# JustinPrivitera/Real_Time_Ray_Tracer

Hardware: AMD Instinct MI355X
Metric: Mrays/s + ms/frame at 3840x2160, 16 AO samples, 64 spheres; 1/2/4/8 GPU (higher is better)
Workload: dtype f32

## Files before the change

### __graft_entry__.py

```python
from __future__ import annotations

import os
import subprocess
import sys
from pathlib import Path

ROOT = Path(__file__).resolve().parent


def build() -> None:
    env = dict(os.environ)
    env.setdefault("PYTORCH_ROCM_ARCH", "gfx950")
    jobs = str(min(16, os.cpu_count() or 1))
    subprocess.run(["make", "-j", jobs, "lib", "headless", "oracle"], cwd=ROOT, check=True, env=env)
    if str(ROOT) not in sys.path:
        sys.path.insert(0, str(ROOT))
    import real_time_ray_tracer_amd as rt

    rt.load()


def smoke() -> None:
    if str(ROOT) not in sys.path:
        sys.path.insert(0, str(ROOT))
    import numpy as np

    import oracle
    import real_time_ray_tracer_amd as rt

    W, H, spp = 64, 48, 4
    h = rt.Header.synthetic(16, spp, 1234, rt.aspect_for(W, H))
    r = rt.Renderer(W, H, h.S, h.AA, device=0)
    ho = h.copy()
    s = rt.SSBO(ho, W, H)
    d = oracle.dims(W, H, h.S, h.AA)
    img = np.zeros((H, W, 4), np.float32)
    fg = fo = 0
    for k in range(3):
        h.fill_rand_buffer(7000 + k)
        h.set_mode(fg, h.num_objects)
        r.upload_header(h)
        fg = r.dispatch(rt.host._lib.RT_MODE_AO_PP, fg)
        s.set_header(h)
        fo = oracle.dispatch(s.data, d, 1, fo, img)
    g = r.download()
    r.close()
    ok = np.abs(g.image - img) <= 1e-4 * np.maximum(np.abs(g.image), np.abs(img)) + 1e-6
    if not ok.all() or fg != fo:
        raise RuntimeError(f"smoke: {int((~ok).sum())} image values differ from the oracle")
    if not np.array_equal(g.depth.view(np.uint32), s.depth.view(np.uint32)):
        raise RuntimeError("smoke: depth g-buffer differs from the oracle")
    print(f"smoke ok: {W}x{H} mode 1, 3 frames, image mean {img[..., :3].mean():.4f}")


if __name__ == "__main__":
    build()
    if len(sys.argv) > 1 and sys.argv[1] == "smoke":
        smoke()
```

### real_time_ray_tracer_amd/csrc/rt_kernels_impl.h

```cpp
#pragma once
#include <hip/hip_runtime.h>

#include "rt_device.h"
#include "rt_kernels.h"

namespace rt {

namespace {

constexpr int kBlock = 256;
constexpr float kGamma = 1.0f / 2.2f;

__device__ __forceinline__ void stage_shapes(const FrameParams& P, float4* lds) {
  const int n = P.nobj;
  for (int k = threadIdx.x; k < 4 * n; k += blockDim.x) {
    int tab = k / n, i = k - tab * n;
    lds[k] = P.shapes[(size_t)tab * P.S + i];
  }
}

__device__ __forceinline__ f3 primary_dir(const FrameParams& P, float hp, float vp) {
  f3 a = mk(P.lx + hp * P.hx, P.ly + hp * P.hy, P.lz + hp * P.hz);
  return normalize(mk(a.x + vp * P.vx, a.y + vp * P.vy, a.z + vp * P.vz));
}
// ... 726 lines not shown
        bounce_round<PL>(P, geo, n, light, live, pos, dir, perm, t, ind, lit);
      }
      if (live) live = !segment(seg, t, ind, lit);
    }
    if (P.tile_cost && (threadIdx.x & 63) == 0)
      P.tile_cost[((unsigned)by * gridDim.x + (unsigned)bx) * (BWX * BWY) + (threadIdx.x >> 6)] = (unsigned)rounds;
  } else {
    for (int seg = 0; active && seg < P.D; ++seg) {
      float t;
      const int ind = closest_hit<ALLSPH>(geo, geo2, n, pos, dir, 0.001f, t);
      const bool lit = ind == -1 || shadow_lit<ALLSPH>(geo, geo2, n, light, pos + t * dir);
      if (segment(seg, t, ind, lit)) break;
    }
  }
  count_work(P, active, y, nseg, nshadow);
  if (active) store_color(P, fd.out_pix, fd.image, x, y, gamma_out(0.0f + rr, 0.0f + rg, 0.0f + rb));
  if (ABL == 7) {
    const unsigned mx = wave_max(active ? nseg : 0u);
    const unsigned long long tend = __builtin_amdgcn_s_memrealtime();
    if ((threadIdx.x & 63) == 0 && active)
      P.out_pix[(size_t)(y - P.band_row0) * P.W + x] =
          make_float4(__uint_as_float((unsigned)tstart), __uint_as_float((unsigned)tend), __uint_as_float(mx),
                      __uint_as_float((unsigned)(tstart >> 32)));
  }
}

template <bool ALLSPH, bool PL = false, bool LT = false, int ABL = 0, int BWX = 2, int BWY = 2, bool MF = true>
__global__ __launch_bounds__(64 * BWX * BWY) void hybrid_kernel(const unsigned* __restrict__ tord,
                                                                const float4* __restrict__ gsph,
                                                                const float4* __restrict__ gshp, unsigned gx,
                                                                FrameParams P) {
  extern __shared__ float4 lds[];
  __shared__ int hperm[64 * BWX * BWY];
  if (!ALLSPH || LT) {
    if (LT) stage_tables(P, lds);
    else stage_shapes(P, lds);
    __syncthreads();
  }
  if constexpr (kHybridTilesPerBlock == 2) {
    const unsigned gx = gridDim.x, gy = (unsigned)(P.trace_rows + 8 * BWY - 1) / (8 * BWY), n = gx * gy;
    const unsigned b = blockIdx.x + blockIdx.y * gx;
#pragma unroll 1
    for (int t = 0; t < 2; ++t) {
      const unsigned u = t == 0 ? b : n - 1 - b;
      if (b > n - 1 - b || (t == 1 && u == b)) break;
      unsigned bx = u % gx, by = u / gx;
      if (tord) {
        const unsigned v = tord[u];
        bx = v & 0xffffu;
        by = v >> 16;
      }
      hybrid_tile<ALLSPH, PL, LT, ABL, BWX, BWY>(P, lds, hperm + 64 * (threadIdx.x >> 6), bx, by, frame_dst(P, blockIdx.z), gsph, gshp);
    }
  } else if constexpr (kHybridTilesPerBlock > 1) {
#pragma unroll 1
    for (int t = 0; t < kHybridTilesPerBlock; ++t)
      hybrid_tile<ALLSPH, PL, LT, ABL, BWX, BWY>(P, lds, hperm + 64 * (threadIdx.x >> 6), blockIdx.x,
                                                 blockIdx.y * kHybridTilesPerBlock + t, frame_dst(P, blockIdx.z), gsph, gshp);
  } else if constexpr (kHybridFramesPerBlock == 1) {
    const bool pre = !MF && ALLSPH && !LT;
    float4 g0;
    if (pre) g0 = gsph[threadIdx.x & 63];
    unsigned bx = blockIdx.x, by = blockIdx.y;
    if (tord) {
      const unsigned t = tord[blockIdx.x + blockIdx.y * gx];
      bx = t & 0xffffu;
      by = t >> 16;
    }
    hybrid_tile<ALLSPH, PL, LT, ABL, BWX, BWY>(P, lds, hperm + 64 * (threadIdx.x >> 6), bx, by,
                                               frame_dst<MF>(P, blockIdx.z), gsph, gshp, pre ? &g0 : nullptr);
  } else {
    int j0;
    const int nj = block_frames<kHybridFramesPerBlock>(P, j0);
#pragma unroll 1
    for (int j = 0; j < nj; ++j)
      hybrid_tile<ALLSPH, PL, LT, ABL, BWX, BWY>(P, lds, hperm + 64 * (threadIdx.x >> 6), blockIdx.x, blockIdx.y,
                                                 frame_dst(P, j0 + j), gsph, gshp);
  }
}

enum { PRIM_HIT = 0, PRIM_MISS = 1, PRIM_EMISSIVE = 2 };

struct BatchLds {
  int prec, sres, pstop, pkind, perm, cmask, rls, geol, total;
};
__host__ __device__ constexpr BatchLds batch_lds(int spp, int pool, int ntail, bool rls_lds = true) {
  const int TP = pool / spp > 0 ? pool / spp : 1, NS = TP * spp;
  BatchLds L{};
  L.prec = 0;
  L.sres = 16 * TP;
  L.pstop = L.sres + 12 * NS;
  L.pkind = L.pstop + 4 * TP;
  L.perm = L.pkind + 4 * ((TP + 1) & ~1);
  L.cmask = (L.perm + 256 + 7) & ~7;
  L.rls = (L.cmask + 8 * 32 + 15) & ~15;
  L.geol = L.rls + (rls_lds ? 32 * spp : 0);
  L.total = L.geol + 16 * ntail;
  return L;
}

#ifndef RT_AO_MINW
#define RT_AO_MINW 7
#endif
#ifndef RT_PT_WIDE
#define RT_PT_WIDE 1
#endif
#ifndef RT_B1_DEFER
#define RT_B1_DEFER 1
#endif
#ifndef RT_B1_PRIO
#define RT_B1_PRIO 1
#endif
#ifndef RT_START_PRIO
#define RT_START_PRIO 1
#endif
#ifndef RT_B1_CREAD
#define RT_B1_CREAD 1
#endif
constexpr int kAoMinWaves = RT_AO_MINW;
template <int MINW, bool LAZY = true, int POOL = kPool, int ABL = 0, bool TAIL = false, bool B1 = false,
          int SPPC = 0, bool PT = false, bool CNT = true, bool PL = false, bool MF = false, bool CL = true, int DC = 0,
          bool CLON = false, bool PTW = false>
__global__ __launch_bounds__(64, MINW) void ao_batch_kernel(FrameParams P, const float4* __restrict__ geo) {
  if (RT_START_PRIO) __builtin_amdgcn_s_setprio(1);
  unsigned long long* const cnts = CNT ? P.counters : nullptr;
  unsigned long long* const rowc = CNT ? P.row_counters : nullptr;
  extern __shared__ float4 lds[];
  const int spp = SPPC ? SPPC : P.spp, W = P.W, D = DC ? DC : P.D, nobj = P.nobj;
  const bool use_cl = CL && (CLON || P.ncl > 0);
  const int fj = MF ? (int)blockIdx.y : 0;
  const int fslot = MF ? (P.mf_slot0 + fj) % P.F : 0;
  float4* const f_nrm = MF ? (float4*)P.hist_nrm[fslot] : P.nrm;
  float4* const f_dep = MF ? (float4*)P.hist_dep[fslot] : P.dep;
  const float4* const f_nrm_prev = MF ? f_nrm : P.nrm_prev;
  const float4* const f_dep_prev = MF ? f_dep : P.dep_prev;
  float4* const f_out = MF ? (float4*)P.hist_pix[fslot] : P.out_pix;
  float4* const f_img = MF ? (fj == P.mf_n - 1 ? P.image : nullptr) : P.image;
  const float4* const f_rb = MF ? P.mf_rb + (size_t)fj * 2 * spp : P.rb;
  const int TP = POOL / spp > 0 ? POOL / spp : 1;
  const int lane = threadIdx.x;
  const int NS = TP * spp;
  const BatchLds LO = batch_lds(spp, POOL, 0, !PTW);
  char* lbase = (char*)lds;
  float4* prec = (float4*)(lbase + LO.prec);
  float* sres = (float*)(lbase + LO.sres);
  int* pstop = (int*)(lbase + LO.pstop);
  int* pkind = (int*)(lbase + LO.pkind);
  int* perm = (int*)(lbase + LO.perm);
  unsigned long long* cmask = (unsigned long long*)(lbase + LO.cmask);
  float4* rls = (float4*)(lbase + LO.rls);
  if (!PTW)
    for (int k = lane; k < 2 * spp; k += 64) rls[k] = f_rb[k];
  for (int k = lane; k < TP; k += 64) pstop[k] = -1;
  float4* geol = (float4*)(lbase + LO.geol);
  constexpr bool tail_lds = TAIL && PT && !PTW;
  const bool tail_ok = TAIL;
  const float4* const tgeo = tail_lds ? geol : geo;
  const bool pt_ok = PT && B1 && (tail_lds || PTW);
  bool geol_valid = false;
  if (tail_lds && !pt_ok) {
    for (int k = lane; k < nobj; k += 64) geol[k] = geo[k];
    geol_valid = true;
  }
  const float4* const clus = geo + (size_t)3 * P.S;
  const unsigned long long* const clm = (const unsigned long long*)(geo + (size_t)3 * P.S + kMaxClusters);
  auto col_at = [&](int ind) -> float4 {
    int o = ind - P.S;
    asm("" : "+v"(o));
    return geo[o - P.S];
  };
  auto aux_at = [&](int ind) -> float4 {
    int o = ind - P.S;
    asm("" : "+v"(o));
    return geo[o];
  };

  const long long npix = (long long)P.trace_rows * W;
  unsigned pb = blockIdx.x;
  if (P.pool_rot > 0) {
    const unsigned Q = (unsigned)P.pool_rot, r = pb / Q;
    if ((r + 1) * Q <= gridDim.x) {
      unsigned c = pb - r * Q + r % Q;
      c = c >= Q ? c - Q : c;
      pb = r * Q + c;
    }
  }
  const long long p0 = (long long)pb * TP;
  const int np = (int)(npix - p0 < TP ? npix - p0 : TP);
  const int total = np * spp;

  unsigned long long tsec[8] = {0, 0, 0, 0, 0, 0, 0, 0};
  constexpr bool kLaps = ABL == 3 || ABL == 6 || ABL == 8;
  unsigned long long tmark = kLaps ? __builtin_amdgcn_s_memtime() : 0;
  auto lap = [&](int k) {
    if (kLaps) {
      unsigned long long now = __builtin_amdgcn_s_memtime();
      tsec[k] += now - tmark;
      tmark = now;
    }
  };
  const int yf = P.trace_row0 + (int)(p0 / W), xf = (int)(p0 % W);
  auto pool_xy = [&](int lp, int& x, int& y) {
    int xi = xf + lp;
    y = yf;
    if (xi >= W) {
      int q = (int)((unsigned)xi / (unsigned)W);
      y += q;
      xi -= q * W;
    }
    x = xi;
  };
  const int yl = P.trace_row0 + (int)((p0 + np - 1) / W), xl = (int)((p0 + np - 1) % W);
  int ncull = 0;
  const int nwords = (nobj + 63) >> 6;
  unsigned long long pmask = 0;
  {
    const ConeF cone = pool_cone_f(P, yf == yl ? xf : 0, yf == yl ? xl : W - 1, yf, yl);
    for (int w = 0; w < nwords; ++w) {
      int i = (w << 6) + lane;
      bool keep = i < nobj && !cone_misses_f(cone, geo[i], P.cx, P.cy, P.cz);
      if (PL) keep = keep && geo[i].x == geo[i].x;
      unsigned long long m = __ballot(keep);
      ncull += __popcll(m);
      if (lane == 0) cmask[w] = m;
    }
    if (PL) {
      pmask = plane_cone_mask(P, cone, mk(P.cx, P.cy, P.cz));
      ncull += __popcll(pmask) + (P.nplanes > 64 ? P.nplanes - 64 : 0);
    }
  }
  __syncthreads();
// ... 40 lines not shown
  unsigned nseg = 0;
  unsigned long long exec_tests = 0;

  const float inv_spp = P.inv_spp;
  auto div_spp = [&](int it) { return SPPC ? (int)((unsigned)it / (unsigned)SPPC) : (int)(((float)it + 0.5f) * inv_spp); };
  auto finish = [&](int it, float r, float g, float b, float stopv, int segs) {
    sres[it] = r;
    sres[NS + it] = g;
    sres[2 * NS + it] = b;
    if (stopv >= 0.0f) {
      const int lq = div_spp(it);
      atomicMax(&pstop[lq], ((it - lq * spp) << 16) | (int)stopv);
    }
    if (rowc) {
      int x, y;
      pool_xy(div_spp(it), x, y);
      atomicAdd(&rowc[y - P.band_row0],
                (unsigned long long)(kSetupCost + ncull + (segs >= 2 ? b1cost + (segs - 2) * nobj : 0)));
    }
  };

  auto shade = [&](int ind, float t, f3& ps, f3& dr, f3 hm, float& r, float& g, float& b, int dpt, int it,
                   bool first) -> bool {
    const int lp = div_spp(it), aa = it - lp * spp;
    float4 att = col_at(ind);
    int kind = PRIM_MISS;
    bool go = false;
    if (ind != -1) {
      const float4 ax = aux_at(ind);
      float4 gc = make_float4(0.0f, 0.0f, 0.0f, 0.0f);
      if (!PL) {
        gc = geo[ind];
        asm volatile("" ::"v"(gc.x), "v"(gc.y), "v"(gc.z));
      }
      if (ax.x > 0.9f) {
        kind = PRIM_EMISSIVE;
      } else {
        kind = PRIM_HIT;
        f3 curr = cam + t * dr;
        f3 nn;
        if (PL) {
          const float4 gi = P.shapes[ind];
          nn = __float_as_int(P.shapes[P.S + ind].w) == SHAPE_PLANE ? xyz(gi) : normalize(curr - xyz(gi));
        } else {
          nn = normalize(curr - xyz(gc));
        }
        if (aa == 0 && first) prec[lp] = make_float4(nn.x, nn.y, nn.z, t);
        if (ABL == 9) {
          float z;
          asm volatile("v_mov_b32 %0, 0" : "=v"(z));
          const f3 c2 = cam + (t + z) * dr;
          const f3 n2 = normalize(c2 - (PL ? xyz(P.shapes[ind]) : xyz(gc)));
          const float d2 = dot(dr, n2);
          const f3 R2 = normalize(mk(dr.x - 2.0f * (d2 * n2.x), dr.y - 2.0f * (d2 * n2.y), dr.z - 2.0f * (d2 * n2.z)));
          const f3 X2 = normalize(ax.y > 0.999f ? hm + n2 : R2 + ax.y * hm);
          if (__float_as_uint(X2.x + X2.y + X2.z) == 0x7fc00001u) t = X2.x;
        }
        ps = curr;
        const float reflect = ax.y;
        f3 X;
        if (reflect > 0.999f) {
          X = hm + nn;
        } else {
          float dn = dot(dr, nn);
          f3 R = normalize(mk(dr.x - 2.0f * (dn * nn.x), dr.y - 2.0f * (dn * nn.y), dr.z - 2.0f * (dn * nn.z)));
          X = R + reflect * hm;
        }
        dr = normalize(X);
        go = dpt - 1 != 0;
      }
    }
    r = r * att.x; g = g * att.y; b = b * att.z;
    if (aa == 0 && first) pkind[lp] = kind;
    if (!go) finish(it, r, g, b, kind == PRIM_HIT ? -1.0f : (float)(D - dpt), kind == PRIM_HIT ? D : D - dpt + 1);
    return go;
  };

  auto prepare = [&]() {
    bitem = next + lane;
    bool live = false;
    if (ABL == 3) { tsec[6] += (unsigned long long)ncull; tsec[7] += 1; }
    exec_tests += (unsigned long long)ncull;
    if (bitem < total) {
      const int lp = div_spp(bitem), aa = bitem - lp * spp;
      int x, y;
      pool_xy(lp, x, y);
      const float px = (float)x, py = (float)y;
      float hp, vp;
      {
        float4 f = rbuf[2 * aa], s = rbuf[2 * aa + 1];
        float uw[2];
        grandom_n<2>({((s.x + px * f.z) - px) + f.x, s.z * px - (f.x * px) * f.z},
                     {((f.y + py * s.w) - py) + s.y, f.w * py - (s.y * py) * s.w}, uw);
        if (ABL == 4) {
          float z, uw2[2];
          asm volatile("v_mov_b32 %0, 0" : "=v"(z));
          grandom_n<2>({((s.x + px * f.z) - px) + f.x + z, s.z * px - (f.x * px) * f.z + z},
                       {((f.y + py * s.w) - py) + s.y, f.w * py - (s.y * py) * s.w}, uw2);
          if (__float_as_uint(uw2[0]) == 0x7fc00001u && __float_as_uint(uw2[1]) == 0x7fc00001u) uw[0] = uw2[0];
        }
        float u = uw[0], w = uw[1];
        normalize2(u, w);
        const float jx = aa == 0 ? 0.0f : div_rn_by(u, 6.0f, kInv6) - 0.08333f;
        const float jy = aa == 0 ? 0.0f : div_rn_by(w, 6.0f, kInv6) - 0.08333f;
        hp = div_rn_by(px + jx, P.fW, P.inv_W);
        vp = div_rn_by(py + jy, P.fH, P.inv_H);
      }
      bdir = primary_dir(P, hp, vp);
      if (ABL == 10) {
        float z;
        asm volatile("v_mov_b32 %0, 0" : "=v"(z));
        float u2 = hp + z, w2 = vp + z;
        normalize2(u2, w2);
        const float jx2 = aa == 0 ? 0.0f : div_rn_by(u2, 6.0f, kInv6) - 0.08333f;
        const float jy2 = aa == 0 ? 0.0f : div_rn_by(w2, 6.0f, kInv6) - 0.08333f;
        const f3 d2 = primary_dir(P, div_rn_by(px + jx2, P.fW, P.inv_W), div_rn_by(py + jy2, P.fH, P.inv_H));
        if (__float_as_uint(d2.x + d2.y + d2.z) == 0x7fc00001u) bdir.x = d2.y;
      }
      auto hemisphere = [&]() {
        float4 f = rbuf[2 * aa], s = rbuf[2 * aa + 1];
        float abe[3];
        grandom_n<3>({f.x + px * s.z, f.z - px * s.z, s.x * px + s.z}, {f.y + py * s.w, f.w - py * s.w, s.y * py + s.w},
                     abe);
        if (ABL == 4) {
          float z, abe2[3];
          asm volatile("v_mov_b32 %0, 0" : "=v"(z));
          grandom_n<3>({f.x + px * s.z + z, f.z - px * s.z + z, s.x * px + s.z + z},
                       {f.y + py * s.w, f.w - py * s.w, s.y * py + s.w}, abe2);
          if (__float_as_uint(abe2[0]) == 0x7fc00001u && __float_as_uint(abe2[2]) == 0x7fc00001u) abe[1] = abe2[1];
        }
        return normalize(mk(abe[0] * 2.0f - 1.0f, abe[1] * 2.0f - 1.0f, abe[2] * 2.0f - 1.0f));
      };
      if (!LAZY) bhemi = hemisphere();
      f3 cv = cam;
      asm("" : "+v"(cv.x), "+v"(cv.y), "+v"(cv.z));
      bpos = cv;
      br = bg = bb = 1.0f;
      float t = -1.0f;
      int ind = -1;
      for (int w = 0; w < nwords; ++w) {
        unsigned long long m = cmask[w];
        m = ((unsigned long long)__builtin_amdgcn_readfirstlane((unsigned)(m >> 32)) << 32) |
            (unsigned)__builtin_amdgcn_readfirstlane((unsigned)m);
        const float4* const gw = geo + (w << 6);
        while (m) {
          const unsigned j = (unsigned)pop_lowest(m);
          const int i = (w << 6) + (int)j;
          sphere_candidate(bpos, bdir, gw[j], i, 0.0001f, t, ind);
          if (ABL == 2) {
            float z;
            asm volatile("v_mov_b32 %0, 0" : "=v"(z));
            float t2 = -1.0f;
            int i2 = -1;
            sphere_candidate(mk(bpos.x + z, bpos.y, bpos.z), bdir, geo[i], i, 0.0001f, t2, i2);
            if (i2 == 0x7fffffff) t = t2;
          }
        }
      }
      if (PL) plane_pass_masked(P, pmask, bpos, bdir, 0.0001f, t, ind);
      ++nseg;
      if (LAZY && ind != -1) bhemi = hemisphere();
      live = shade(ind, t, bpos, bdir, bhemi, br, bg, bb, D, bitem, true);
    }
    bdepth = D - 1;
    b1cost = nobj;
    if (B1) {
      const unsigned long long lm1 = __ballot(live);
      if (lm1 != 0 && __popcll(lm1) >= P.b1_min) {
        lap(1);
        if (RT_B1_PRIO) __builtin_amdgcn_s_setprio(1);
        const ConeB cb = bounce_cone(live, bpos, bdir, lm1);
        float t = -1.0f;
        int ind = -1;
        b1cost = 0;
        if (ABL == 12) {
          float z;
          asm volatile("v_mov_b32 %0, 0" : "=v"(z));
          const ConeB c2 = bounce_cone(live, mk(bpos.x + z, bpos.y, bpos.z), bdir, lm1);
          unsigned long long acc = 0;
          for (int w = 0; w < nwords; ++w) {
            const int i = (w << 6) + lane_id_here();
            float4 pt;
            const bool k2 = i < nobj && bounce_cone_keep_pt(c2, geo[i], pt);
            acc ^= __ballot(k2 && pt.w != 7.0f);
          }
          if (acc == 0x123456789abcdefull) b1cost = 1;
        }
        unsigned long long ru = 0;
        int ksel = 0;
        f3 tdir = bdir;
        if (RT_B1_DEFER && !live) tdir = mk(__int_as_float(0x7fc00000), __int_as_float(0x7fc00000), __int_as_float(0x7fc00000));
        auto flush = [&]() {
          const float4 gs = geo[ksel];
          sphere_candidate_if(bpos, bdir, gs, ksel, 0.0001f, t, ind, ru);
          ru = 0;
        };
        for (int w = 0; w < nwords; ++w) {
          const int i = (w << 6) + lane_id_here();
          bool keep;
          if (pt_ok) {
            float4 pt;
            keep = i < nobj && bounce_cone_keep_pt(cb, geo[i], pt);
            if (i < nobj) geol[PTW ? i - (w << 6) : i] = pt;
          } else {
            keep = i < nobj && !bounce_cone_misses(cb, geo[i]);
          }
          if (PL) keep = keep && geo[i].x == geo[i].x;
          unsigned long long m = __ballot(keep);
          m = ((unsigned long long)__builtin_amdgcn_readfirstlane((unsigned)(m >> 32)) << 32) |
              (unsigned)__builtin_amdgcn_readfirstlane((unsigned)m);
          exec_tests += (unsigned long long)__popcll(m);
          b1cost += __popcll(m);
          if (ABL == 3) tsec[6] += (unsigned long long)__popcll(m) << 24;
          if (pt_ok) {
            geol_valid = false;
            __syncthreads();
            if (ABL == 6) lap(5);
            const float4* const qw = geol + (PTW ? 0 : (w << 6));
            const float4* const gw = geo + (w << 6);
            int qbase;
            asm("v_mov_b32 %0, %1" : "=v"(qbase) : "s"((int)(size_t)((const char*)qw - lbase)));
            if (RT_B1_DEFER || live)
              while (m) {
                const int j = pop_lowest(m), k = (w << 6) + j;
#if RT_B1_CREAD
                const float4 q = *(const float4*)(lbase + (qbase + (j << 4)));
#else
                typedef float v4f __attribute__((ext_vector_type(4)));
                v4f qv;
                int j_addr_scratch;
                asm volatile("v_lshl_add_u32 %1, %2, 4, %3\n\tds_read_b128 %0, %1\n\ts_waitcnt lgkmcnt(0)"
                             : "=v"(qv), "=&v"(j_addr_scratch)
                             : "s"(j), "v"(qbase));
                const float4 q = make_float4(qv.x, qv.y, qv.z, qv.w);
#endif
                const float4 g = gw[j];
                if (ABL == 7) {
                  const bool pass = fmaf(bdir.z, q.z, fmaf(bdir.y, q.y, bdir.x * q.x)) >= q.w;
                  const f3 pmc = bpos - xyz(g);
                  const float bb = dot(bdir, pmc);
                  const float del = fmaf(g.w, g.w, fmaf(bb, bb, -dot(pmc, pmc)));
                  const unsigned long long pm = __ballot(pass), dm = __ballot(pass && del >= 0.0f);
                  tsec[0] += 1; tsec[1] += pm != 0; tsec[2] += dm != 0;
                  tsec[3] += (unsigned long long)__popcll(pm);
                }
                const bool pass = fmaf(tdir.z, q.z, fmaf(tdir.y, q.y, tdir.x * q.x)) >= q.w;
                if (ABL == 5) {
                  float z, t2 = t;
                  int i2 = ind;
                  asm volatile("v_mov_b32 %0, 0" : "=v"(z));
                  const bool pass2 = fmaf(bdir.z + z, q.z, fmaf(bdir.y, q.y, bdir.x * q.x)) >= q.w;
                  const unsigned long long pm2 = __builtin_amdgcn_ballot_w64(pass2);
                  if (pm2 != 0) sphere_candidate_if(mk(bpos.x + z, bpos.y, bpos.z), bdir, g, k, 0.0001f, t2, i2, pm2);
                  if (i2 == 0x7fffffff) t = t2;
                }
                const unsigned long long pm = __builtin_amdgcn_ballot_w64(pass);
                if (RT_B1_DEFER) {
                  if (pm != 0) {
                    if (pm & ru) flush();
                    ru |= pm;
                    int kv = k;
                    asm("v_cndmask_b32_e64 %0, %1, %2, %3" : "=v"(ksel) : "v"(ksel), "v"(kv), "s"(pm));
                  }
                } else if (pm != 0) {
                  sphere_candidate_if(bpos, bdir, g, k, 0.0001f, t, ind, pm);
                }
              }
            if (ABL == 6) lap(6);
          } else if (live) {
            while (m) {
              const int k = (w << 6) + __builtin_ctzll(m);
              m &= m - 1;
              sphere_candidate(bpos, bdir, geo[k], k, 0.0001f, t, ind);
            }
          }
        }
        if (RT_B1_DEFER && ru != 0) flush();
        if (RT_B1_PRIO) __builtin_amdgcn_s_setprio(0);
        if (ABL == 7) { tsec[4] += 1; tsec[5] += (unsigned long long)__popcll(lm1); }
        if (live) {
          if (PL) plane_pass(P, bpos, bdir, 0.0001f, t, ind);
          ++nseg;
          live = shade(ind, t, bpos, bdir, bhemi, br, bg, bb, D - 1, bitem, false);
        }
        if (ABL == 6) lap(7);
        bdepth = D - 2;
        lap(4);
      }
    }
    unsigned long long lm = __ballot(live);
    if (live) perm[__builtin_amdgcn_mbcnt_hi((unsigned)(lm >> 32), __builtin_amdgcn_mbcnt_lo((unsigned)lm, 0u))] = lane;
    nlive = __popcll(lm);
    cursor = 0;
    next = next + 64 < total ? next + 64 : total;
    __syncthreads();
  };

  for (;;) {
    for (;;) {
      unsigned long long need = __ballot(!has);
      if (need == 0) break;
      if (cursor >= nlive) {
        if (next >= total) break;
        lap(2);
        prepare();
        lap(1);
        continue;
      }
      int r = __builtin_amdgcn_mbcnt_hi((unsigned)(need >> 32), __builtin_amdgcn_mbcnt_lo((unsigned)need, 0u));
      int take = __popcll(need) < nlive - cursor ? __popcll(need) : nlive - cursor;
      bool get = !has && r < take;
      int src = get ? perm[cursor + r] : lane;
      float sx = __shfl(bpos.x, src), sy = __shfl(bpos.y, src), sz = __shfl(bpos.z, src);
      float dx = __shfl(bdir.x, src), dy = __shfl(bdir.y, src), dz = __shfl(bdir.z, src);
      float hx = __shfl(bhemi.x, src), hy = __shfl(bhemi.y, src), hz = __shfl(bhemi.z, src);
      float cr = __shfl(br, src), cg = __shfl(bg, src), cb = __shfl(bb, src);
      int ci = __shfl(bitem, src);
      if (ABL == 11) {
        int zi;
        asm volatile("v_mov_b32 %0, 0" : "=v"(zi));
        const int s2 = src + zi;
        float q = __shfl(bpos.x, s2) + __shfl(bpos.y, s2) + __shfl(bpos.z, s2) + __shfl(bdir.x, s2) + __shfl(bdir.y, s2) +
                  __shfl(bdir.z, s2) + __shfl(bhemi.x, s2) + __shfl(bhemi.y, s2) + __shfl(bhemi.z, s2) + __shfl(br, s2) +
                  __shfl(bg, s2) + __shfl(bb, s2) + (float)__shfl(bitem, s2);
        if (__float_as_uint(q) == 0x7fc00001u) cr = q;
      }
      if (get) {
        pos = mk(sx, sy, sz);
        dir = mk(dx, dy, dz);
        hemi = mk(hx, hy, hz);
        rr = cr; rg = cg; rb = cb;
        item = ci;
        depth = bdepth;
        has = true;
      }
      cursor += take;
    }
    const unsigned long long hm = __ballot(has);
    if (hm == 0) break;
    lap(2);
    if (ABL == 3) tsec[5] += 1;
    const int L = __popcll(hm);
    if (tail_ok && next >= total && cursor >= nlive && L <= 32) {
      if (tail_lds && !geol_valid) {
        __syncthreads();
        for (int k = lane_id_here(); k < nobj; k += 64) geol[k] = geo[k];
        geol_valid = true;
      }
      int c = 0;
      while ((1 << c) < L) ++c;
      const int G = 64 >> c;
      const int rk = __builtin_amdgcn_mbcnt_hi((unsigned)(hm >> 32), __builtin_amdgcn_mbcnt_lo((unsigned)hm, 0u));
      if (has) perm[rk] = lane;
      __syncthreads();
      const int g = lane / G, pl = lane - g * G;
      const bool act = g < L;
      const int owner = act ? perm[g] : lane;
      const f3 o = mk(__shfl(pos.x, owner), __shfl(pos.y, owner), __shfl(pos.z, owner));
      const f3 d = mk(__shfl(dir.x, owner), __shfl(dir.y, owner), __shfl(dir.z, owner));
      float t = -1.0f;
      int ind = -1;
      if (use_cl && G <= kClusterTailMaxG) {
        unsigned long long kc = 0;
        for (int c0 = 0; c0 < P.ncl; c0 += G) {
          const int c = c0 + pl;
          const bool may = act && c < P.ncl && cluster_may_hit(o, d, clus[c]);
          unsigned long long b = __builtin_amdgcn_ballot_w64(may);
          for (int sh = 32; sh >= G; sh >>= 1) b |= b >> sh;
          kc |= (G == 64 ? b : (b & ((1ull << G) - 1))) << c0;
        }
        unsigned char* list = (unsigned char*)cmask;
        int cnt = 0;
        for (int w = 0; w < nwords; ++w) {
          unsigned long long m = clm[w];
          for (unsigned long long k2 = kc; k2;) m |= clm[(size_t)(1 + pop_lowest(k2)) * kClusterWords + w];
          const int ln = lane_id_here();
          if ((m >> ln) & 1ull)
            list[cnt + __builtin_amdgcn_mbcnt_hi((unsigned)(m >> 32), __builtin_amdgcn_mbcnt_lo((unsigned)m, 0u))] =
                (unsigned char)((w << 6) + ln);
          cnt += __popcll(m);
// ... 377 lines not shown
    case 9: out[i] = det_sin(__uint_as_float(__float_as_uint(in[0]) + (unsigned)i)); break;
    case 1: out[i] = grandom(in[2 * i], in[2 * i + 1]); break;
    case 2: out[i] = sqrt_rn(in[i]); break;
    case 6: {
      const unsigned per = (unsigned)in[0];
      unsigned bad = 0;
      for (unsigned k = 0; k < per; ++k) {
        unsigned long long u = (unsigned long long)i * per + k;
        if (u > 0x7f800000ull) break;
        float x = __uint_as_float((unsigned)u);
        bad += __float_as_uint(sqrt_rn(x)) != __float_as_uint(sqrtf(x));
      }
      out[i] = (float)bad;
      break;
    }
    case 7: {
      const unsigned per = (unsigned)in[0];
      unsigned bad = 0;
      for (unsigned k = 0; k < per; ++k) {
        unsigned long long u = (unsigned long long)i * per + k;
        if (u > 0x7f800000ull) break;
        float x = __uint_as_float((unsigned)u);
        bad += __float_as_uint(inv_len_rn(x)) != __float_as_uint(1.0f / sqrtf(x));
        if (u >= 0x00800000ull && u <= 0x7e800000ull) bad += __float_as_uint(rcp_rn_normal(x)) != __float_as_uint(1.0f / x);
      }
      out[i] = (float)bad;
      break;
    }
    case 8: {
      const unsigned per = (unsigned)in[0];
      unsigned bad = 0;
      for (unsigned k = 0; k < per; ++k) {
        unsigned long long u = (unsigned long long)i * per + k;
        if (u > 0x7f7fffffull) break;
        float x = __uint_as_float((unsigned)u);
        const float s = sqrt_rn_tail(x);
        if (u >= 0x0f800000ull) bad += __float_as_uint(s) != __float_as_uint(sqrtf(x));
        else bad += !(s >= 0.0f && s <= 0x1p-47f);
      }
      out[i] = (float)bad;
      break;
    }
    case 3: out[i] = in[2 * i] / in[2 * i + 1]; break;
    case 11: {
      if (i < (size_t)kSinTableN) {
        const float x = __uint_as_float(kSinTableX[i]);
        out[2 * i] = sin_ambiguous(sin_binary64(x)) ? 1.0f : 0.0f;
        out[2 * i + 1] = __uint_as_float(kSinTableX[i]);
      } else {
        out[2 * i] = -1.0f;
        out[2 * i + 1] = 0.0f;
      }
      break;
    }
    case 10: {
      const f3 lv = mk(in[4 * i], in[4 * i + 1], in[4 * i + 2]);
      const f3 l = normalize(lv);
      const float len = sqrtf(dot(lv, lv));
      const bool occ = shadow_occludes(in[4 * i + 3], l, (double)len, shadow_bounds(l, len));
      out[5 * i] = l.x; out[5 * i + 1] = l.y; out[5 * i + 2] = l.z; out[5 * i + 3] = len;
      out[5 * i + 4] = occ ? 1.0f : 0.0f;
      break;
    }
    case 4: {
      f3 v = normalize(mk(in[3 * i], in[3 * i + 1], in[3 * i + 2]));
      out[3 * i] = v.x; out[3 * i + 1] = v.y; out[3 * i + 2] = v.z;
      break;
    }
    case 5: {
      const float* a = in + 10 * i;
      out[i] = sphere_eval(mk(a[0], a[1], a[2]), mk(a[3], a[4], a[5]), make_float4(a[6], a[7], a[8], a[9]));
      break;
    }
    default: break;
  }
}

size_t shapes_lds_bytes(const FrameParams& p) { return (size_t)4 * p.nobj * sizeof(float4); }
size_t tab_lds_bytes(const FrameParams& p) { return (size_t)5 * (p.nobj > 0 ? p.nobj : 1) * sizeof(float4); }

}

constexpr int kRefDepth = 20;

template <int SPPC, bool PL, int DC = 0, bool CLON = false>
inline void launch_batch(bool tl, bool cnt, dim3 g, dim3 b, size_t lds, hipStream_t stream, const FrameParams& q) {
  constexpr bool GT = RT_GLOBAL_TAIL;
  constexpr bool TLC = RT_TL_CLUSTERS;
  constexpr bool PTWV = RT_PT_WIDE;
  if (q.mf_n > 0) {
    g.y = (unsigned)q.mf_n;
    if (tl)
      hipLaunchKernelGGL((ao_batch_kernel<kAoMinWaves, true, kPool, 0, true, true, SPPC, true, false, PL, true, TLC, DC, CLON>), g, b, lds, stream, q, q.sph);
    else
      hipLaunchKernelGGL((ao_batch_kernel<kAoMinWaves, true, kPool, 0, GT, true, SPPC, PTWV, false, PL, true, true, DC, CLON, PTWV>), g, b, lds, stream, q, q.sph);
    return;
  }
  if (tl && cnt)
    hipLaunchKernelGGL((ao_batch_kernel<kAoMinWaves, true, kPool, 0, true, true, SPPC, true, true, PL, false, TLC, DC, CLON>), g, b, lds, stream, q, q.sph);
  else if (tl)
    hipLaunchKernelGGL((ao_batch_kernel<kAoMinWaves, true, kPool, 0, true, true, SPPC, true, false, PL, false, TLC, DC, CLON>), g, b, lds, stream, q, q.sph);
  else if (cnt)
    hipLaunchKernelGGL((ao_batch_kernel<kAoMinWaves, true, kPool, 0, GT, true, SPPC, PTWV, true, PL, false, true, DC, CLON, PTWV>), g, b, lds, stream, q, q.sph);
  else
    hipLaunchKernelGGL((ao_batch_kernel<kAoMinWaves, true, kPool, 0, GT, true, SPPC, PTWV, false, PL, false, true, DC, CLON, PTWV>), g, b, lds, stream, q, q.sph);
}

__global__ __launch_bounds__(256) void gbuf_convert_kernel(GbufXfer x) {
  const size_t total = (size_t)x.F * x.W * x.R;
  const size_t idx = (size_t)blockIdx.x * 256 + threadIdx.x;
  if (idx >= total) return;
  const size_t wr = (size_t)x.W * x.R;
  const int f = (int)(idx / wr);
  const size_t rem = idx - (size_t)f * wr;
  const int xx = (int)(rem / x.R), r = (int)(rem - (size_t)xx * x.R);
  const size_t o = (size_t)(x.r0 + r) * x.W + xx;
  float4* base = x.slot[f];
  if (x.to_ref) {
    x.ref[idx] = x.kind == 0 ? base[o] : x.kind == 1 ? nrm_load(base, x.n, o) : dep_load(base, x.n, o);
  } else {
    const float4 v = x.ref[idx];
    if (x.kind == 0) base[o] = v;
    else if (x.kind == 1) nrm_store(base, x.n, o, v);
    else dep_store(base, x.n, o, v);
  }
}

inline hipError_t launch_gbuf_convert_impl(const GbufXfer& x, hipStream_t stream) {
  const size_t total = (size_t)x.F * x.W * x.R;
  if (total == 0) return hipSuccess;
  hipLaunchKernelGGL(gbuf_convert_kernel, dim3((unsigned)((total + 255) / 256)), dim3(256), 0, stream, x);
  return hipGetLastError();
}

inline FrameParams launch_params(const FrameParams& p) {
  FrameParams q = p;
  q.sph = p.shapes + sphere_table(p.S);
  q.planes = p.shapes + plane_table(p.S);
  q.clus = p.shapes + cluster_table(p.S);
  q.clmask = (const unsigned long long*)(p.shapes + cluster_mask_table(p.S));
  q.camrel = p.shapes + camrel_table(p.S);
  q.b1_min = 1;
  {
    const int TP = kPool / p.spp > 0 ? kPool / p.spp : 1;
    const int ppr = p.W / TP;
    q.pool_rot = ppr >= 8 ? ppr : 8;
  }
  {
    const int gx = (p.W + kPostTileW - 1) / kPostTileW;
    int R = 0;
    if (gx % 8 == 0)
      for (int r = 4; r <= gx / 16 && !R; ++r)
        if ((gx / 8) % r == 0) R = r;
    q.tile_run = R ? R : (gx >= 32 ? 4 : 0);
#ifdef RT_POST_RUN
    q.tile_run = RT_POST_RUN;
#endif
    const int gy = (p.trace_rows + kPostTileH - 1) / kPostTileH;
    q.post_sx = gx % 4 == 0 ? 4 : (gx % 2 == 0 ? 2 : 1);
    q.post_sy = gy % 4 == 0 ? 4 : (gy % 2 == 0 ? 2 : 1);
    if (gx < 8 * q.post_sx) q.post_sx = q.post_sy = 1;
  }
  return q;
}

inline hipError_t launch_production(int program, const FrameParams& p, const FrameParams& q, hipStream_t stream) {
  const bool pl = p.nplanes > 0;
  if (program == K_AOP || program == K_AO) {
    const long long npix = (long long)p.trace_rows * p.W;
    const int TP = kPool / p.spp > 0 ? kPool / p.spp : 1;
    const long long pools = (npix + TP - 1) / TP;
    const bool tl = p.nobj <= kTailMaxObj;
    const size_t psh = (size_t)batch_lds(p.spp, kPool, tl ? p.nobj : (RT_PT_WIDE ? 64 : 0), tl || !RT_PT_WIDE).total;
    const dim3 g((unsigned)pools), b(64);
    const bool cnt = p.counters || p.row_counters;
    if (!pl) {
      const bool ref_d = p.D == kRefDepth && p.ncl > 0;
      if (p.spp == 16 && ref_d) launch_batch<16, false, kRefDepth, true>(tl, cnt, g, b, psh, stream, q);
      else if (p.spp == 64 && ref_d) launch_batch<64, false, kRefDepth, true>(tl, cnt, g, b, psh, stream, q);
      else if (p.spp == 16) launch_batch<16, false>(tl, cnt, g, b, psh, stream, q);
      else if (p.spp == 64) launch_batch<64, false>(tl, cnt, g, b, psh, stream, q);
      else if (p.spp == 4) launch_batch<4, false>(tl, cnt, g, b, psh, stream, q);
      else launch_batch<0, false>(tl, cnt, g, b, psh, stream, q);
    } else {
      if (p.spp == 16) launch_batch<16, true>(tl, cnt, g, b, psh, stream, q);
      else if (p.spp == 4) launch_batch<4, true>(tl, cnt, g, b, psh, stream, q);
      else launch_batch<0, true>(tl, cnt, g, b, psh, stream, q);
    }
    return hipGetLastError();
  }
  const int fpb = program == K_PHONG ? kPhongFramesPerBlock : kHybridFramesPerBlock;
  const int tpb = program == K_HYBRID ? kHybridTilesPerBlock : 1;
  const int tw = program == K_HYBRID ? kHyTile : 16;
  dim3 grid((p.W + tw - 1) / tw, ((p.trace_rows + tw - 1) / tw + tpb - 1) / tpb, p.mf_n > 0 ? (p.mf_n + fpb - 1) / fpb : 1);
  const dim3 hyb(64 * kHyBW * kHyBW);
#ifndef RT_HY_NOLT
#define RT_HY_NOLT 1
#endif
#ifndef RT_PH_NOLT
#define RT_PH_NOLT 1
#endif
  const bool lt = p.nobj <= kTabLdsMax && !(RT_HY_NOLT && program == K_HYBRID) && !(RT_PH_NOLT && program == K_PHONG);
  const size_t ltb = lt ? tab_lds_bytes(p) : 0;
  const bool mf = p.mf_n > 0;
  switch (program) {
    case K_PHONG:
      if (pl && lt) hipLaunchKernelGGL((phong_kernel<true, true, true>), grid, dim3(kBlock), ltb, stream, q.sph, q.shapes, q);
      else if (pl && mf) hipLaunchKernelGGL((phong_kernel<true, true, false>), grid, dim3(kBlock), 0, stream, q.sph, q.shapes, q);
      else if (pl) hipLaunchKernelGGL((phong_kernel<true, true, false, false>), grid, dim3(kBlock), 0, stream, q.sph, q.shapes, q);
      else if (lt) hipLaunchKernelGGL((phong_kernel<true, false, true>), grid, dim3(kBlock), ltb, stream, q.sph, q.shapes, q);
      else if (mf) hipLaunchKernelGGL((phong_kernel<true, false, false>), grid, dim3(kBlock), 0, stream, q.sph, q.shapes, q);
      else hipLaunchKernelGGL((phong_kernel<true, false, false, false>), grid, dim3(kBlock), 0, stream, q.sph, q.shapes, q);
      break;
    case K_HYBRID:
      if (pl && lt) hipLaunchKernelGGL((hybrid_kernel<true, true, true, 0, kHyBW, kHyBW>), grid, hyb, ltb, stream, q.tile_order, q.sph, q.shapes, grid.x, q);
      else if (pl && mf) hipLaunchKernelGGL((hybrid_kernel<true, true, false, 0, kHyBW, kHyBW>), grid, hyb, 0, stream, q.tile_order, q.sph, q.shapes, grid.x, q);
      else if (pl) hipLaunchKernelGGL((hybrid_kernel<true, true, false, 0, kHyBW, kHyBW, false>), grid, hyb, 0, stream, q.tile_order, q.sph, q.shapes, grid.x, q);
      else if (lt) hipLaunchKernelGGL((hybrid_kernel<true, false, true, 0, kHyBW, kHyBW>), grid, hyb, ltb, stream, q.tile_order, q.sph, q.shapes, grid.x, q);
      else if (mf) hipLaunchKernelGGL((hybrid_kernel<true, false, false, 0, kHyBW, kHyBW>), grid, hyb, 0, stream, q.tile_order, q.sph, q.shapes, grid.x, q);
      else hipLaunchKernelGGL((hybrid_kernel<true, false, false, 0, kHyBW, kHyBW, false>), grid, hyb, 0, stream, q.tile_order, q.sph, q.shapes, grid.x, q);
      break;
    case K_POST:
      hipLaunchKernelGGL(post_kernel,
                         dim3((p.W + kPostTileW - 1) / kPostTileW, (p.trace_rows + kPostTileH - 1) / kPostTileH),
                         dim3(kBlock), 0, stream, q);
      break;
    default:
      return hipErrorInvalidValue;
  }
  return hipGetLastError();
}

inline hipError_t launch_selftest_impl(int fn, const float* d_in, float* d_out, size_t n, hipStream_t stream) {
  if (n == 0) return hipSuccess;
  unsigned grid = (unsigned)((n + 255) / 256);
  hipLaunchKernelGGL(selftest_kernel, dim3(grid), dim3(256), 0, stream, fn, d_in, d_out, n);
  return hipGetLastError();
}

}
```

Baseline: 62020.

## Sort AO hemisphere rays by octant in LDS before batch tracing

```diff
diff --git a/__graft_entry__.py b/__graft_entry__.py
--- a/__graft_entry__.py
+++ b/__graft_entry__.py
@@ -12,7 +12,7 @@
     env = dict(os.environ)
     env.setdefault("PYTORCH_ROCM_ARCH", "gfx950")
     jobs = str(min(16, os.cpu_count() or 1))
-    subprocess.run(["make", "-j", jobs, "lib", "headless", "oracle"], cwd=ROOT, check=True, env=env)
+    subprocess.run(["make", "-j", jobs, "lib", "headless", "oracle", "b1sort0"], cwd=ROOT, check=True, env=env)
     if str(ROOT) not in sys.path:
         sys.path.insert(0, str(ROOT))
     import real_time_ray_tracer_amd as rt
diff --git a/real_time_ray_tracer_amd/csrc/rt_kernels_impl.h b/real_time_ray_tracer_amd/csrc/rt_kernels_impl.h
--- a/real_time_ray_tracer_amd/csrc/rt_kernels_impl.h
+++ b/real_time_ray_tracer_amd/csrc/rt_kernels_impl.h
@@ -832,9 +832,9 @@
 enum { PRIM_HIT = 0, PRIM_MISS = 1, PRIM_EMISSIVE = 2 };
 
 struct BatchLds {
-  int prec, sres, pstop, pkind, perm, cmask, rls, geol, total;
+  int prec, sres, pstop, pkind, perm, order, cmask, rls, geol, total;
 };
-__host__ __device__ constexpr BatchLds batch_lds(int spp, int pool, int ntail, bool rls_lds = true) {
+__host__ __device__ constexpr BatchLds batch_lds(int spp, int pool, int ntail, bool rls_lds = true, bool sort = false) {
   const int TP = pool / spp > 0 ? pool / spp : 1, NS = TP * spp;
   BatchLds L{};
   L.prec = 0;
@@ -842,7 +842,8 @@
   L.pstop = L.sres + 12 * NS;
   L.pkind = L.pstop + 4 * TP;
   L.perm = L.pkind + 4 * ((TP + 1) & ~1);
-  L.cmask = (L.perm + 256 + 7) & ~7;
+  L.order = L.perm + 256;
+  L.cmask = (L.order + (sort ? pool : 0) + 7) & ~7;
   L.rls = (L.cmask + 8 * 32 + 15) & ~15;
   L.geol = L.rls + (rls_lds ? 32 * spp : 0);
   L.total = L.geol + 16 * ntail;
@@ -867,10 +868,13 @@
 #ifndef RT_B1_CREAD
 #define RT_B1_CREAD 1
 #endif
+#ifndef RT_B1_SORT
+#define RT_B1_SORT 1
+#endif
 constexpr int kAoMinWaves = RT_AO_MINW;
 template <int MINW, bool LAZY = true, int POOL = kPool, int ABL = 0, bool TAIL = false, bool B1 = false,
           int SPPC = 0, bool PT = false, bool CNT = true, bool PL = false, bool MF = false, bool CL = true, int DC = 0,
-          bool CLON = false, bool PTW = false>
+          bool CLON = false, bool PTW = false, bool SORT = false>
 __global__ __launch_bounds__(64, MINW) void ao_batch_kernel(FrameParams P, const float4* __restrict__ geo) {
   if (RT_START_PRIO) __builtin_amdgcn_s_setprio(1);
   unsigned long long* const cnts = CNT ? P.counters : nullptr;
@@ -890,13 +894,15 @@
   const int TP = POOL / spp > 0 ? POOL / spp : 1;
   const int lane = threadIdx.x;
   const int NS = TP * spp;
-  const BatchLds LO = batch_lds(spp, POOL, 0, !PTW);
+  static_assert(!SORT || (LAZY && POOL % 64 == 0 && POOL <= 256), "SORT: hemi is read back from LDS; items are bytes");
+  const BatchLds LO = batch_lds(spp, POOL, 0, !PTW, SORT);
   char* lbase = (char*)lds;
   float4* prec = (float4*)(lbase + LO.prec);
   float* sres = (float*)(lbase + LO.sres);
   int* pstop = (int*)(lbase + LO.pstop);
   int* pkind = (int*)(lbase + LO.pkind);
   int* perm = (int*)(lbase + LO.perm);
+  unsigned char* order = (unsigned char*)(lbase + LO.order);
   unsigned long long* cmask = (unsigned long long*)(lbase + LO.cmask);
   float4* rls = (float4*)(lbase + LO.rls);
   if (!PTW)
@@ -1103,6 +1109,7 @@
     if (ABL == 3) { tsec[6] += (unsigned long long)ncull; tsec[7] += 1; }
     exec_tests += (unsigned long long)ncull;
     if (bitem < total) {
+      if (SORT) bitem = order[bitem];
       const int lp = div_spp(bitem), aa = bitem - lp * spp;
       int x, y;
       pool_xy(lp, x, y);
@@ -1180,7 +1187,7 @@
       }
       if (PL) plane_pass_masked(P, pmask, bpos, bdir, 0.0001f, t, ind);
       ++nseg;
-      if (LAZY && ind != -1) bhemi = hemisphere();
+      if (LAZY && ind != -1) bhemi = SORT ? mk(sres[bitem], sres[NS + bitem], sres[2 * NS + bitem]) : hemisphere();
       live = shade(ind, t, bpos, bdir, bhemi, br, bg, bb, D, bitem, true);
     }
     bdepth = D - 1;
@@ -1317,6 +1324,78 @@
     __syncthreads();
   };
 
+  if (SORT) {
+    constexpr int NC = POOL / 64, NF = 3;
+    static_assert(NC * (1 << NF) <= 64, "one cell per lane");
+    const int ln = lane_id_here();
+    perm[ln] = 0;
+    __syncthreads();
+    int key[NC];
+#pragma unroll
+    for (int c = 0; c < NC; ++c) {
+      key[c] = 0;
+      if (c * 64 < total) {
+        const int it = c * 64 + ln;
+        f3 h = mk(0.0f, 0.0f, 0.0f);
+        if (it < total) {
+          const int lp = div_spp(it), aa = it - lp * spp;
+          int x, y;
+          pool_xy(lp, x, y);
+          const float px = (float)x, py = (float)y;
+          const float4 f = rbuf[2 * aa], s = rbuf[2 * aa + 1];
+          float abe[3];
+          grandom_n<3>({f.x + px * s.z, f.z - px * s.z, s.x * px + s.z}, {f.y + py * s.w, f.w - py * s.w, s.y * py + s.w},
+                       abe);
+          h = normalize(mk(abe[0] * 2.0f - 1.0f, abe[1] * 2.0f - 1.0f, abe[2] * 2.0f - 1.0f));
+          sres[it] = h.x;
+          sres[NS + it] = h.y;
+          sres[2 * NS + it] = h.z;
+        }
+        const int nv = total - c * 64;
+        const unsigned long long mv = nv >= 64 ? ~0ull : (1ull << nv) - 1;
+        unsigned own_lo = (unsigned)mv, own_hi = (unsigned)(mv >> 32);
+        unsigned oct = 0;
+        const float hc[NF] = {h.x, h.y, h.z};
+#pragma unroll
+        for (int k = NF - 1; k >= 0; --k) {
+          const int bits = __float_as_int(hc[k]);
+          const unsigned long long m = __ballot(bits < 0);
+          const unsigned sgn = (unsigned)(bits >> 31);
+          own_lo &= ~((unsigned)m ^ sgn);
+          own_hi &= ~((unsigned)(m >> 32) ^ sgn);
+          oct = oct << 1 | (unsigned)bits >> 31;
+        }
+        const int cell = (int)oct * NC + c;
+        const int r = (int)__builtin_amdgcn_mbcnt_hi(own_hi, __builtin_amdgcn_mbcnt_lo(own_lo, 0u));
+        if (it < total) perm[cell] = __popc(own_lo) + __popc(own_hi);
+        key[c] = r | cell << 8;
+      }
+    }
+    __syncthreads();
+    {
+      const int bin = ln / NC, c = ln % NC;
+      const bool in = ln < NC * (1 << NF);
+      const int cell = in ? (bin ^ (bin >> 1)) * NC + c : 0;
+      const int n = in ? perm[cell] : 0;
+      int acc = n;
+      acc += __builtin_amdgcn_update_dpp(0, acc, 0x111, 0xf, 0xf, false);
+      acc += __builtin_amdgcn_update_dpp(0, acc, 0x112, 0xf, 0xf, false);
+      acc += __builtin_amdgcn_update_dpp(0, acc, 0x114, 0xf, 0xf, false);
+      acc += __builtin_amdgcn_update_dpp(0, acc, 0x118, 0xf, 0xf, false);
+      acc += __builtin_amdgcn_update_dpp(0, acc, 0x142, 0xa, 0xf, false);
+      acc += __builtin_amdgcn_update_dpp(0, acc, 0x143, 0xc, 0xf, false);
+      __syncthreads();
+      if (in) perm[cell] = acc - n;
+    }
+    __syncthreads();
+#pragma unroll
+    for (int c = 0; c < NC; ++c) {
+      const int it = c * 64 + ln;
+      if (it < total) order[perm[key[c] >> 8] + (key[c] & 255)] = (unsigned char)it;
+    }
+    __syncthreads();
+  }
+
   for (;;) {
     for (;;) {
       unsigned long long need = __ballot(!has);
@@ -1860,8 +1939,12 @@
 }
 
 constexpr int kRefDepth = 20;
-
-template <int SPPC, bool PL, int DC = 0, bool CLON = false>
+#ifndef RT_B1_SORT_MIN
+#define RT_B1_SORT_MIN 48
+#endif
+constexpr int kB1SortMinObj = RT_B1_SORT_MIN;
+
+template <int SPPC, bool PL, int DC = 0, bool CLON = false, bool SORT = false>
 inline void launch_batch(bool tl, bool cnt, dim3 g, dim3 b, size_t lds, hipStream_t stream, const FrameParams& q) {
   constexpr bool GT = RT_GLOBAL_TAIL;
   constexpr bool TLC = RT_TL_CLUSTERS;
@@ -1869,19 +1952,19 @@
   if (q.mf_n > 0) {
     g.y = (unsigned)q.mf_n;
     if (tl)
-      hipLaunchKernelGGL((ao_batch_kernel<kAoMinWaves, true, kPool, 0, true, true, SPPC, true, false, PL, true, TLC, DC, CLON>), g, b, lds, stream, q, q.sph);
+      hipLaunchKernelGGL((ao_batch_kernel<kAoMinWaves, true, kPool, 0, true, true, SPPC, true, false, PL, true, TLC, DC, CLON, false, SORT>), g, b, lds, stream, q, q.sph);
     else
-      hipLaunchKernelGGL((ao_batch_kernel<kAoMinWaves, true, kPool, 0, GT, true, SPPC, PTWV, false, PL, true, true, DC, CLON, PTWV>), g, b, lds, stream, q, q.sph);
+      hipLaunchKernelGGL((ao_batch_kernel<kAoMinWaves, true, kPool, 0, GT, true, SPPC, PTWV, false, PL, true, true, DC, CLON, PTWV, SORT>), g, b, lds, stream, q, q.sph);
     return;
   }
   if (tl && cnt)
-    hipLaunchKernelGGL((ao_batch_kernel<kAoMinWaves, true, kPool, 0, true, true, SPPC, true, true, PL, false, TLC, DC, CLON>), g, b, lds, stream, q, q.sph);
+    hipLaunchKernelGGL((ao_batch_kernel<kAoMinWaves, true, kPool, 0, true, true, SPPC, true, true, PL, false, TLC, DC, CLON, false, SORT>), g, b, lds, stream, q, q.sph);
   else if (tl)
-    hipLaunchKernelGGL((ao_batch_kernel<kAoMinWaves, true, kPool, 0, true, true, SPPC, true, false, PL, false, TLC, DC, CLON>), g, b, lds, stream, q, q.sph);
+    hipLaunchKernelGGL((ao_batch_kernel<kAoMinWaves, true, kPool, 0, true, true, SPPC, true, false, PL, false, TLC, DC, CLON, false, SORT>), g, b, lds, stream, q, q.sph);
   else if (cnt)
-    hipLaunchKernelGGL((ao_batch_kernel<kAoMinWaves, true, kPool, 0, GT, true, SPPC, PTWV, true, PL, false, true, DC, CLON, PTWV>), g, b, lds, stream, q, q.sph);
+    hipLaunchKernelGGL((ao_batch_kernel<kAoMinWaves, true, kPool, 0, GT, true, SPPC, PTWV, true, PL, false, true, DC, CLON, PTWV, SORT>), g, b, lds, stream, q, q.sph);
   else
-    hipLaunchKernelGGL((ao_batch_kernel<kAoMinWaves, true, kPool, 0, GT, true, SPPC, PTWV, false, PL, false, true, DC, CLON, PTWV>), g, b, lds, stream, q, q.sph);
+    hipLaunchKernelGGL((ao_batch_kernel<kAoMinWaves, true, kPool, 0, GT, true, SPPC, PTWV, false, PL, false, true, DC, CLON, PTWV, SORT>), g, b, lds, stream, q, q.sph);
 }
 
 __global__ __launch_bounds__(256) void gbuf_convert_kernel(GbufXfer x) {
@@ -1949,10 +2032,20 @@
     const int TP = kPool / p.spp > 0 ? kPool / p.spp : 1;
     const long long pools = (npix + TP - 1) / TP;
     const bool tl = p.nobj <= kTailMaxObj;
-    const size_t psh = (size_t)batch_lds(p.spp, kPool, tl ? p.nobj : (RT_PT_WIDE ? 64 : 0), tl || !RT_PT_WIDE).total;
+    const bool sort = RT_B1_SORT && !pl && p.nobj >= kB1SortMinObj;
+    const size_t psh =
+        (size_t)batch_lds(p.spp, kPool, tl ? p.nobj : (RT_PT_WIDE ? 64 : 0), tl || !RT_PT_WIDE, sort).total;
     const dim3 g((unsigned)pools), b(64);
     const bool cnt = p.counters || p.row_counters;
-    if (!pl) {
+    if (sort) {
+      const bool ref_d = p.D == kRefDepth && p.ncl > 0;
+      if (p.spp == 16 && ref_d) launch_batch<16, false, kRefDepth, true, RT_B1_SORT != 0>(tl, cnt, g, b, psh, stream, q);
+      else if (p.spp == 64 && ref_d) launch_batch<64, false, kRefDepth, true, RT_B1_SORT != 0>(tl, cnt, g, b, psh, stream, q);
+      else if (p.spp == 16) launch_batch<16, false, 0, false, RT_B1_SORT != 0>(tl, cnt, g, b, psh, stream, q);
+      else if (p.spp == 64) launch_batch<64, false, 0, false, RT_B1_SORT != 0>(tl, cnt, g, b, psh, stream, q);
+      else if (p.spp == 4) launch_batch<4, false, 0, false, RT_B1_SORT != 0>(tl, cnt, g, b, psh, stream, q);
+      else launch_batch<0, false, 0, false, RT_B1_SORT != 0>(tl, cnt, g, b, psh, stream, q);
+    } else if (!pl) {
       const bool ref_d = p.D == kRefDepth && p.ncl > 0;
       if (p.spp == 16 && ref_d) launch_batch<16, false, kRefDepth, true>(tl, cnt, g, b, psh, stream, q);
       else if (p.spp == 64 && ref_d) launch_batch<64, false, kRefDepth, true>(tl, cnt, g, b, psh, stream, q);
```

Result: faster. 63840 (median of 6 runs) (+2.9%).
